# facebookresearch/hanabi_SAD

Hardware: AMD Instinct MI355X
Metric: hanabi_env_steps_per_sec (higher is better)
Workload: dtype u32

## Files before the change

hanabi_sad_amd/csrc/hsad_env.hip:

```cpp

#include <hip/hip_runtime.h>

#include <cstdarg>
#include <cstdlib>
#include <cstdio>
#include <cstring>
#include <new>
#include <string>
#include <vector>

#include "hsad.h"
#include "hsad_deal_fast.h"
#include "hsad_obs_row.h"
#include "hsad_planes.h"

namespace {

constexpr int kWave = 64;
constexpr int kMtN = 624;
constexpr int kMtM = 397;

struct EnvParams {
  static constexpr bool kScripted = false;
  int G, Gpad, P, H, A, F, F0, LAL, OB, OD, OL, OK, DECKW;
// ... 782 lines not shown
  return m;
}

template <int TH, class Ru>
__device__ __forceinline__ uint64_t legal_mask_of(int P, int H, int A, const uint32_t* s_st, int lane, int p, uint32_t pm,
                                                  const Ru& ru) {
  const uint32_t board = ST(PL_BOARD);
  const int cur = board_cur(board), info = board_info(board);
  uint64_t lm = 0;
  if (p == cur) {
    const uint32_t hw = ST(PLH(p));
    const int len = (hw >> 25) & 7;
    const uint64_t lenmask = (1ull << len) - 1ull;
    if (info < ru.MI) lm |= lenmask;
    lm |= lenmask << H;
    if (info > 0) {
      for (int o = 1; o < P; ++o) {
        int q = p + o;
        if (q >= P) q -= P;
        const uint32_t thw = ST(PLH(q));
        const int tl = (thw >> 25) & 7;
        uint32_t cm = 0, rm = 0;
#pragma unroll
        for (int i = 0; i < (TH ? TH : 5); ++i) {
          const int card = (thw >> (5 * i)) & 31;
          const int c = (card * 13) >> 6, r = card - 5 * c;
          if (i < tl) {
            cm |= 1u << perm_c(pm, c);
            rm |= 1u << r;
          }
        }
        lm |= (uint64_t)cm << (2 * H + (o - 1) * ru.C);
        lm |= (uint64_t)rm << (2 * H + (P - 1) * ru.C + (o - 1) * ru.R);
      }
    }
  }
  if (!lm) lm = 1ull << (A - 1);
  return lm;
}

template <int TP, int TH, bool V = false, bool FIXED = false>
__device__ __forceinline__ void build_rows(const EnvParams& ep, const uint32_t* s_st, int lane, int g, uint32_t* s_obs,
                                           uint32_t* s_legal, uint32_t* s_own, uint32_t greedy_rec, int p_begin,
                                           int p_step, uint32_t* s_lmask = nullptr) {
  const int P = TP ? TP : ep.P, H = TH ? TH : ep.H;
  const auto ru = RulesOf<V>::make(ep);
  const uint32_t CR = (uint32_t)ru.CR, RR = (uint32_t)ru.R;
  const uint32_t board = ST(PL_BOARD);
  const uint32_t misc = ST(PL_MISC);
  const int deck_size = (misc >> 8) & 63;
  const uint64_t disc = (uint64_t)ST(PL_DISC_LO) | ((uint64_t)ST(PL_DISC_HI) << 32);
  const uint32_t lastmv = ST(PL_LASTMV);
  const int info = board_info(board), life = board_life(board);
  const uint32_t F = (uint32_t)ep.F;

  for (int p = p_begin; p < P; p += p_step) {
    const uint32_t base = (uint32_t)(lane * P + p) * F;
    const uint32_t pm = ep.shuffle_color ? (ST(PLPERM(p)) & 0x7fffu) : kIdentityPerm;
    if constexpr (FIXED) {
      static_assert(TP > 0 && TH > 0 && !V, "fixed bit positions need a fixed game shape and the full rules");
      uint32_t hand[TP], kcp[TP], krp[TP], kh[TP];
#pragma unroll
      for (int o = 0; o < TP; ++o) {
        int q = p + o;
        if (q >= P) q -= P;
        hand[o] = ST(PLH(q));
        kcp[o] = ST(PLKCP(q));
        krp[o] = ST(PLKRP(q));
        kh[o] = ST(PLKH(q));
      }
      uint32_t row[ObsRowGeom<TP, TH>::NW];
      obs_row_assemble<TP, TH>(row, board, misc, disc, lastmv, greedy_rec, hand, kcp, krp, kh, p, pm, ep.sad != 0);
      obs_row_place<TP, TH>(row, base, ep.sad != 0, [s_obs](uint32_t w, uint32_t v) { atomicOr(&s_obs[w], v); });
    } else {
      uint32_t miss = 0;
#pragma unroll
      for (int o = 0; o < (TP ? TP : 5); ++o) {
        if (o >= P) break;
        int q = p + o;
        if (q >= P) q -= P;
        const uint32_t hw = ST(PLH(q));
        const int len = (hw >> 25) & 7;
        if (len < H) miss |= 1u << o;
        const uint32_t kcp = ST(PLKCP(q)), krp = ST(PLKRP(q)), kh = ST(PLKH(q));
#pragma unroll
        for (int i = 0; i < (TH ? TH : 5); ++i) {
          if (i < len) {
            if (o > 0) {
              const int card = (hw >> (5 * i)) & 31;
              const int c = (card * 13) >> 6, r = card - 5 * c;
              or_bit(s_obs, base + (uint32_t)((o * H + i) * ru.CR) + perm_c(pm, c) * RR + (uint32_t)r);
            }
            const uint32_t cp = (kcp >> (5 * i)) & 31u, rp = (krp >> (5 * i)) & 31u;
            const uint32_t h6 = (kh >> (6 * i)) & 63u;
            uint64_t m = 0;
#pragma unroll
            for (int c = 0; c < 5; ++c) m |= ((cp >> c) & 1u) ? ((uint64_t)rp << (perm_c(pm, c) * RR)) : 0ull;
            if (h6 & 7u) m |= 1ull << (CR + perm_c(pm, (int)(h6 & 7u) - 1));
            if (h6 >> 3) m |= 1ull << (CR + (uint32_t)ru.C + (h6 >> 3) - 1u);
            or_bits64(s_obs, base + (uint32_t)ep.OK + (uint32_t)((o * H + i) * ru.KS), m);
          }
        }
      }
      or_bits32(s_obs, base + (uint32_t)(P * H * ru.CR), miss);
      or_bits64(s_obs, base + (uint32_t)ep.OB, (1ull << deck_size) - 1ull);
      uint64_t bm = 0;
#pragma unroll
      for (int c = 0; c < 5; ++c) {
        const int f = board_fw(board, c);
        bm |= (f > 0) ? (1ull << (perm_c(pm, c) * RR + (uint32_t)f - 1u)) : 0ull;
      }
      bm |= (uint64_t)((1u << info) - 1u) << CR;
      bm |= (uint64_t)((1u << life) - 1u) << (CR + (uint32_t)ru.MI);
      or_bits64(s_obs, base + (uint32_t)(ep.OB + ep.DECKW), bm);
      uint64_t dm = 0;
#pragma unroll
      for (int c = 0; c < 5; ++c) {
        const uint32_t pc = perm_c(pm, c);
#pragma unroll
        for (int r = 0; r < 5; ++r) {
          const uint32_t n = cnt2(disc, c * 5 + r);
          const uint32_t roff = (r == 0) ? 0u : (1u + 2u * (uint32_t)r);
          dm |= (uint64_t)((1u << n) - 1u) << (pc * (uint32_t)ru.DW + roff);
        }
      }
      or_bits64(s_obs, base + (uint32_t)ep.OD, dm);
      or_bits64(s_obs, base + (uint32_t)ep.OL, encode_last_action(P, H, lastmv, p, pm, ru));
      if (ep.sad) or_bits64(s_obs, base + (uint32_t)ep.F0, encode_last_action(P, H, greedy_rec, p, pm, ru));
    }

    const uint64_t lm = legal_mask_of<TH>(P, H, ep.A, s_st, lane, p, pm, ru);
    or_bits64(s_legal, (uint32_t)(lane * P + p) * (uint32_t)ep.A, lm);
    ep.legal_bits[(size_t)g * P + p] = lm;
    if (ep.legal_out) ep.legal_out[(size_t)g * P + p] = lm;
    if (s_lmask) {
      s_lmask[(2 * p) * kWave + lane] = (uint32_t)lm;
      s_lmask[(2 * p + 1) * kWave + lane] = (uint32_t)(lm >> 32);
    }

    {
      const uint32_t hw = ST(PLH(p));
      const int len = (hw >> 25) & 7;
      uint32_t om = 0;
#pragma unroll
      for (int i = 0; i < (TH ? TH : 5); ++i) {
        const int card = (hw >> (5 * i)) & 31;
        const int c = (card * 13) >> 6, r = card - 5 * c;
        const int f = board_fw(board, c);
        if (i < len) om |= 1u << (3 * i + (r == f ? 0 : (r < f ? 1 : 2)));
      }
      or_bits32(s_own, (uint32_t)(lane * P + p) * (uint32_t)(3 * H), om);
      if (ep.own_bits) ep.own_bits[(size_t)g * P + p] = om;
    }
  }
}

__device__ __forceinline__ uint64_t public_counts(uint64_t disc, uint32_t board, uint64_t full) {
  uint64_t pc = full - disc;
#pragma unroll
  for (int c = 0; c < 5; ++c) {
    const int f = board_fw(board, c);
    for (int r = 0; r < f; ++r) pc -= (uint64_t)1 << (2 * (c * 5 + r));
  }
  return pc;
}

template <bool V>
__device__ void v0_fixup(const EnvParams& ep, const uint32_t* s_st, const uint32_t* s_obs, uint64_t active, int g0,
                         int lane_id) {
  const int P = ep.P, H = ep.H;
  const auto ru = RulesOf<V>::make(ep);
  const int per_row = P * H * ru.CR;
  while (active) {
    const int lg = __builtin_ctzll(active);
    active &= active - 1;
    const uint32_t board = s_st[PL_BOARD * kWave + lg];
    const uint64_t disc = (uint64_t)s_st[PL_DISC_LO * kWave + lg] | ((uint64_t)s_st[PL_DISC_HI * kWave + lg] << 32);
    const uint64_t pub = public_counts(disc, board, ru.full);
    for (int e = lane_id; e < P * per_row; e += kWave) {
      const int p = e / per_row;
      const int rem = e - p * per_row;
      const int slot = rem / ru.CR;
      const int j = rem - slot * ru.CR;
      const int o = slot / H, i = slot - o * H;
      int q = p + o;
      if (q >= P) q -= P;
      const uint32_t hw = s_st[PLH(q) * kWave + lg];
      if (i >= (int)((hw >> 25) & 7)) continue;
      const uint32_t bitpos = (uint32_t)(lg * P + p) * (uint32_t)ep.F + (uint32_t)ep.OK + (uint32_t)(slot * ru.KS + j);
      if (!get1(s_obs, bitpos)) continue;
      const uint32_t permw = ep.shuffle_color ? s_st[PLPERM(p) * kWave + lg] : kIdentityPermBoth;
      const uint32_t inv = permw >> 15;
      const uint32_t cp = (s_st[PLKCP(q) * kWave + lg] >> (5 * i)) & 31u;
      const uint32_t rp = (s_st[PLKRP(q) * kWave + lg] >> (5 * i)) & 31u;
      float total = 0.f;
      for (int c = 0; c < 5; ++c)
        if ((cp >> c) & 1u)
          for (int r = 0; r < 5; ++r)
            if ((rp >> r) & 1u) total += (float)cnt2(pub, c * 5 + r);
      const int pcol = j / ru.R, r = j - ru.R * pcol;
      const int real_c = (int)perm_c(inv, pcol);
      const float cnt = (float)cnt2(pub, real_c * 5 + r);
      const float v = (total > 0.f) ? cnt / total : 0.f;
      ep.priv_s[(size_t)(g0 + lg) * P * ep.F + (size_t)p * ep.F + ep.OK + slot * ru.KS + j] = v;
    }
  }
}

__device__ __forceinline__ void log_error(const EnvParams& ep, int g, int code) {
  if (atomicAdd(&ep.err[0], 1u) == 0u) {
    ep.err[1] = (uint32_t)g;
    ep.err[2] = (uint32_t)code;
  }
}

__device__ __forceinline__ int policy_pick(uint64_t seed, uint64_t game, uint64_t counter, int p, int stream,
                                           uint64_t mask) {
  const uint32_t h = policy_hash(seed, game, counter, (uint64_t)(p * 2 + stream));
  return df_select(mask, h % (uint32_t)__popcll(mask));
}
__device__ __forceinline__ uint64_t policy_key(uint64_t seed, uint64_t game, int p, int stream) {
  return mix64(seed ^ mix64(game * 0xD1342543DE82EF95ull + (uint64_t)(p * 2 + stream)));
}
__device__ __forceinline__ int policy_pick_keyed(uint64_t key, uint64_t counter, uint64_t mask, int nbits) {
  const uint32_t h = (uint32_t)(mix64(key + counter) >> 32);
  return df_select(mask, h % (uint32_t)__popcll(mask), nbits);
}

constexpr int kEnvThreads = 4 * kWave;

__device__ __forceinline__ void stream_rows(const EnvParams& ep, const uint32_t* s_obs, const uint32_t* s_legal, const uint32_t* s_own,
                                            int g0, int ng, int P, int H, int t, int n) {
  const size_t PF = (size_t)P * ep.F, PA = (size_t)P * ep.A, PO = (size_t)P * 3 * H;
  if (!ep.obs_f32) {
  } else if (ep.nt_stores) {
    stream_bits_f32_aligned<true>(s_obs, ep.priv_s + (size_t)g0 * PF, (uint32_t)(ng * PF), t, n);
  } else {
    stream_bits_f32_aligned<false>(s_obs, ep.priv_s + (size_t)g0 * PF, (uint32_t)(ng * PF), t, n);
  }
  stream_rows_packed(ep, s_obs, 0, ng * P, (size_t)g0 * P, t, n);
  stream_bits_f32_aligned<false>(s_legal, ep.legal + (size_t)g0 * PA, (uint32_t)(ng * PA), t, n);
  stream_bits_f32_aligned<false>(s_own, ep.own + (size_t)g0 * PO, (uint32_t)(ng * PO), t, n);
}

__device__ __forceinline__ unsigned stream_rows_delta(const EnvParams& ep, const uint32_t* s_obs, uint32_t* s_old, bool all,
                                                      const uint32_t* s_legal, const uint32_t* s_own, int g0, int ng, int P, int H,
                                                      int t, int n, bool count, int compact, unsigned& units) {
  const size_t PF = (size_t)P * ep.F, PA = (size_t)P * ep.A, PO = (size_t)P * 3 * H;
  unsigned stored = 0;
  bool by_lines = true;
  if (!ep.obs_f32) {
  } else if (compact && !all) {
    by_lines = false;
    float* out = ep.priv_s + (size_t)g0 * PF;
    if (compact == 2) {
      if (ep.nt_stores) {
        stored = stream_bits_f32_compact<true, 16>(s_obs, s_old, out, (uint32_t)(ng * PF), t, units);
      } else {
        stored = stream_bits_f32_compact<false, 16>(s_obs, s_old, out, (uint32_t)(ng * PF), t, units);
      }
    } else if (ep.nt_stores) {
      stored = stream_bits_f32_compact<true, 32>(s_obs, s_old, out, (uint32_t)(ng * PF), t, units);
    } else {
      stored = stream_bits_f32_compact<false, 32>(s_obs, s_old, out, (uint32_t)(ng * PF), t, units);
    }
  } else if (ep.nt_stores) {
    stored = stream_bits_f32_delta<true>(s_obs, s_old, all, ep.priv_s + (size_t)g0 * PF, (uint32_t)(ng * PF), t, n, count);
  } else {
    stored = stream_bits_f32_delta<false>(s_obs, s_old, all, ep.priv_s + (size_t)g0 * PF, (uint32_t)(ng * PF), t, n, count);
  }
  if (by_lines) units = stored;
  stream_rows_packed(ep, s_obs, 0, ng * P, (size_t)g0 * P, t, n);
  stream_bits_f32_aligned<false>(s_legal, ep.legal + (size_t)g0 * PA, (uint32_t)(ng * PA), t, n);
  stream_bits_f32_aligned<false>(s_own, ep.own + (size_t)g0 * PO, (uint32_t)(ng * PO), t, n);
  return stored;
}

__device__ __forceinline__ void clear_words(uint32_t* p, int nz, int t, int n) {
  uint4* z4 = reinterpret_cast<uint4*>(p);
  for (int k = t; k < (nz >> 2); k += n) z4[k] = make_uint4(0u, 0u, 0u, 0u);
  for (int k = (nz & ~3) + t; k < nz; k += n) p[k] = 0u;
}

__device__ __forceinline__ void clear_rows(const EnvParams& ep, uint32_t* s_obs, int t, int n) {
  const int nz = ep.obs_words + ep.legal_words + ep.own_words;
  uint4* z4 = reinterpret_cast<uint4*>(s_obs);
  for (int k = t; k < (nz >> 2); k += n) z4[k] = make_uint4(0u, 0u, 0u, 0u);
  for (int k = (nz & ~3) + t; k < nz; k += n) s_obs[k] = 0u;
}

struct LogicCarry {
  uint32_t* counter;
  const uint32_t* s_lmask;
  const uint64_t* pkey;
};
template <int TP, int TH>
constexpr bool kPolicyKeys = (TP == 2 && TH == 5);
template <int N>
__device__ __forceinline__ uint64_t carried_key(const uint64_t* k, int i) {
  uint64_t v = k[0];
#pragma unroll
  for (int j = 1; j < N; ++j) v = (i == j) ? k[j] : v;
  return v;
}
typedef __attribute__((address_space(3))) const uint32_t* LdsWordPtr;

// ... 425 lines not shown

  Rng rng;
  rng.mt = ep.mt + (size_t)g * kMtN;
  rng.draws = ST(PL_DRAWS);
  rng.la0 = ST(PL_LA0);
  rng.la1 = ST(PL_LA1);
  rng.la_n = (int)((ST(PL_MISC) >> 22) & 3u);
  rng.spos = (rng.draws + (uint32_t)rng.la_n) % (uint32_t)kMtN;
  rng.win = nullptr;
  rng.w_c = rng.w_n = 0;
  uint32_t greedy_rec = 0;
  float reward = 0.f;
  bool term = false;

  if (wave == 0) {
    env_logic<MODE, TP, TH, V>(ep, a_in, g_in, s_st, s_win, s_eps, lane, g, active, do_reset, rng, greedy_rec, reward, term, dbg_it);
    s_grec[lane] = greedy_rec;
  }
  __syncthreads();
  STAMP(2);

  Refill rf;
  refill_issue(rf, rng, active && wave == 0);
  if (active) build_rows<TP, TH, V>(ep, s_st, lane, g, s_obs, s_legal, s_own, s_grec[lane], wave, nwaves);
  STAMP(3);
  if (active && wave == 0) {
    refill_finish(rf, rng);
    ST(PL_DRAWS) = rng.draws;
    ST(PL_LA0) = rng.la0;
    ST(PL_LA1) = rng.la1;
    ST(PL_MISC) = (ST(PL_MISC) & ~(3u << 22)) | ((uint32_t)rng.la_n << 22);
    for (int pl = 0; pl < ep.npl; ++pl) ep.planes[(size_t)pl * ep.Gpad + g] = ST(pl);
  }
  __syncthreads();
  STAMP(4);

  const size_t PF = (size_t)P * ep.F, PA = (size_t)P * ep.A, PO = (size_t)P * 3 * H;
  if (MODE >= 1) {
    stream_rows(ep, s_obs, s_legal, s_own, g0, ng, P, H, tid, nthreads);
    if (valid && wave == 0) {
      for (int p = 0; p < P; ++p) ep.eps[(size_t)g * P + p] = __uint_as_float(ST(PLEPS(p)));
      ep.reward[g] = reward;
      ep.terminal[g] = term ? 1 : 0;
    }
    if (ep.kmode == 1) {
      __syncthreads();
      if (wave == 0) v0_fixup<V>(ep, s_st, s_obs, __ballot(valid), g0, lane);
    }
  } else {
    if (wave != 0) return;
    uint64_t todo = __ballot(active);
    const uint64_t todo_all = todo;
    while (todo) {
      const int lg = __builtin_ctzll(todo);
      todo &= todo - 1;
      if (ep.obs_f32) stream_bits_f32(s_obs, (uint32_t)(lg * PF), ep.priv_s + (size_t)(g0 + lg) * PF, (uint32_t)PF, lane);
      stream_rows_packed(ep, s_obs, lg * P, P, (size_t)(g0 + lg) * P, lane, kWave);
      stream_bits_f32(s_legal, (uint32_t)(lg * PA), ep.legal + (size_t)(g0 + lg) * PA, (uint32_t)PA, lane);
      stream_bits_f32(s_own, (uint32_t)(lg * PO), ep.own + (size_t)(g0 + lg) * PO, (uint32_t)PO, lane);
    }
    if (active)
      for (int p = 0; p < P; ++p) ep.eps[(size_t)g * P + p] = __uint_as_float(ST(PLEPS(p)));
    if (ep.kmode == 1) {
      __syncthreads();
      v0_fixup<V>(ep, s_st, s_obs, todo_all, g0, lane);
    }
  }
  STAMP(5);
}

template <int MODE, int TP, int TH, bool V = false>
__global__ __launch_bounds__(kEnvThreads) void env_kernel(EnvParams ep, const int64_t* __restrict__ a_in,
                                                          const int64_t* __restrict__ g_in) {
  env_body<MODE, TP, TH, V>(ep, a_in, g_in);
}

template <int TP, int TH, bool V = false>
__global__ __launch_bounds__(kEnvThreads) void env_step_scripted_kernel(ScriptedParams ep, const int64_t* __restrict__ a_in,
                                                                        const int64_t* __restrict__ g_in) {
  env_body<1, TP, TH, V>(ep, a_in, g_in);
}

__device__ __forceinline__ void rollout_stagger(const EnvParams& ep) {
  if (ep.stagger_ticks > 0) {
    unsigned k = blockIdx.x & 7u;
    if (ep.stagger_mode == 1) k = ((blockIdx.x >> 3) >> 5) & 3u;
    else if (ep.stagger_mode == 2) k = (blockIdx.x >> 3) & 3u;
    else if (ep.stagger_mode == 3) {
      unsigned hw;
      asm volatile("s_getreg_b32 %0, hwreg(HW_REG_HW_ID)" : "=s"(hw));
      k = (hw & 15u) >> 1;
    }
    const unsigned long long t_in = wall_clock64(), wait = (unsigned long long)k * (unsigned long long)ep.stagger_ticks;
    while (wall_clock64() - t_in < wait) __builtin_amdgcn_s_sleep(16);
  }
}

__device__ __forceinline__ unsigned pace_delay(const EnvParams& ep, unsigned long long s, int iter, unsigned t_own) {
  const long long num = (long long)iter * ep.pace_blocks - (long long)(s - ep.pace_base);
  const long long span = (long long)ep.n_iter * ep.pace_blocks;
  if (num < -span || num > span) return 0u;
  const int over_q8 = (int)((num * (long long)ep.pace_inv_q32) >> 24) - ep.pace_l0_q8;
  if (over_q8 <= 0) return 0u;
  t_own = min(t_own, 1u << 20);
  const unsigned long long d = ((unsigned long long)(unsigned)over_q8 * t_own) >> 8;
  return (unsigned)min(d, (unsigned long long)min(t_own >> 1, (unsigned)ep.pace_cap_ticks));
}

__device__ __forceinline__ unsigned long long pace_count(const EnvParams& ep) {
  int z = 0;
  unsigned long long one = 1ull;
  asm volatile("" : "+v"(z), "+v"(one));
  return __hip_atomic_fetch_add(ep.pace + z, one, __ATOMIC_RELAXED, __HIP_MEMORY_SCOPE_AGENT);
}

__device__ __forceinline__ void pace_sleep(unsigned ticks) {
  const unsigned long long t_in = wall_clock64();
  while (wall_clock64() - t_in < (unsigned long long)ticks) __builtin_amdgcn_s_sleep(16);
}

template <int TP, int TH, bool V = false>
__global__ __launch_bounds__(kEnvThreads) __attribute__((amdgpu_waves_per_eu(2, 2))) void env_rollout_kernel(EnvParams ep) {
  rollout_stagger(ep);
  unsigned long long pace_s = 0ull;
  unsigned pace_t0 = (unsigned)wall_clock64();
  const bool paced = ep.pace && ep.g_begin + (int)blockIdx.x * ep.gpw < ep.G;
#pragma clang loop unroll(disable)
  for (int iter = 0; iter < ep.n_iter; ++iter) {
    if (iter) __syncthreads();
    if (paced) {
      const unsigned now = (unsigned)wall_clock64(), t_own = now - pace_t0;
      pace_t0 = now;
      if (threadIdx.x == 0) {
        if (iter > 0) {
          const unsigned d = pace_delay(ep, pace_s, iter - 1, t_own);
          if (d) pace_sleep(d);
        }
        pace_s = pace_count(ep);
      }
    }
    int zero = 0;
    asm volatile("" : "+s"(zero));
    env_body<3, TP, TH, V>(ep, nullptr, nullptr, zero, iter);
  }
}

#ifdef HSAD_ENV_ROWBUILD_SCATTER
template <int TP, int TH>
constexpr bool kRowBuildFixed = false;
#else
template <int TP, int TH>
constexpr bool kRowBuildFixed = TP > 0 && TH > 0;
#endif

__device__ __forceinline__ unsigned wave_sum(unsigned v) {
  for (int o = kWave / 2; o > 0; o >>= 1) v += (unsigned)__shfl_xor((int)v, o, kWave);
  return v;
}

constexpr int kChainIn = 2, kChainOut = 4;
__device__ __forceinline__ uint4* chain_slice(const EnvParams& ep) {
  return reinterpret_cast<uint4*>(reinterpret_cast<uint32_t*>(ep.phase) + (size_t)blockIdx.x * ep.obs_words);
}

template <int TP, int TH>
__global__ __launch_bounds__(kEnvThreads) __attribute__((amdgpu_waves_per_eu(2, 2))) void env_rollout_pipe_kernel(EnvParams ep) {
  if constexpr (kRowBuildFixed<TP, TH>) asm volatile("" ::: "v175");
  rollout_stagger(ep);
  extern __shared__ __attribute__((aligned(16))) uint32_t smem[];
  uint32_t* s_st = smem;
  uint32_t* s_obs = s_st + ep.npl * kWave;
  uint32_t* s_legal = s_obs + ep.obs_words;
  uint32_t* s_own = s_legal + ep.legal_words;
  uint32_t* s_win = s_own + ep.own_words;
  uint32_t* s_grec = s_win + ep.win_words * kWave;
  float* s_eps = reinterpret_cast<float*>(s_grec + kWave);
  uint32_t* s_pace = s_grec + kWave + 128;
#define S_OBS1(z) (ep.delta ? s_pace + 4 + (z) : s_obs)

  const int tid = threadIdx.x;
  const int lane = tid & (kWave - 1);
  const int wave = tid >> 6;
  const int g0 = ep.g_begin + blockIdx.x * ep.gpw;
  const int ng = min(ep.gpw, ep.G - g0);
  if (ng <= 0) return;
  const int P = TP ? TP : ep.P, H = TH ? TH : ep.H;

  uint32_t act_counter = 0u;
  uint64_t pkey[kPolicyKeys<TP, TH> ? 2 * TP : 1] = {};
  if (wave == 0) {
    const int g = g0 + lane;
    if (lane < ng) {
      act_counter = ep.act_count[g];
      if constexpr (kPolicyKeys<TP, TH>) {
#pragma unroll
        for (int k = 0; k < 2 * TP; ++k) pkey[k] = policy_key(ep.policy_seed, (uint64_t)g, k >> 1, k & 1);
      }
      for (int p = 0; p < P; ++p) {
        const uint64_t lm = ep.legal_bits[(size_t)g * P + p];
        s_win[(2 * p) * kWave + lane] = (uint32_t)lm;
        s_win[(2 * p + 1) * kWave + lane] = (uint32_t)(lm >> 32);
      }
    }
    for (int pl0 = 0; pl0 < ep.npl; pl0 += 8) {
      uint32_t v[8];
#pragma unroll
      for (int j = 0; j < 8; ++j) v[j] = ep.planes[(size_t)min(pl0 + j, ep.npl - 1) * ep.Gpad + g];
#pragma unroll
      for (int j = 0; j < 8; ++j)
        if (pl0 + j < ep.npl) ST(pl0 + j) = v[j];
    }
  } else {
    clear_rows(ep, s_obs, lane, kWave);
    if (ep.delta & kChainIn) {
      const uint4* src = chain_slice(ep);
      uint4* dst = reinterpret_cast<uint4*>(S_OBS1(0));
      for (int k = lane; k < (ep.obs_words >> 2); k += kWave) dst[k] = src[k];
    }
    for (int k = lane; k < min(ep.n_eps, 128); k += kWave) s_eps[k] = ep.eps_list[k];
    if (lane == 0) s_pace[0] = 0u;
  }
  __syncthreads();

  unsigned pace_t0 = (unsigned)wall_clock64();
#pragma clang loop unroll(disable)
  for (int iter = 0; iter < ep.n_iter; ++iter) {
    int zero = 0;
    asm volatile("" : "+s"(zero));
    const int g = g0 + zero + lane;
    const bool valid = lane < ep.gpw && g < ep.G;
    const int dbg_it = iter;
    STAMP_START();
    unsigned long long pace_s = 0ull;
    if (ep.pace && tid == 0) pace_s = pace_count(ep);
    const unsigned pace_now = (unsigned)wall_clock64(), pace_t_own = pace_now - pace_t0;
    pace_t0 = pace_now;
    Rng rng = {};
    float reward = 0.f;
    bool term = false;
    if (wave == 0) {
      if (ep.dbg && ep.dbg_iters > 0) {
        asm volatile("s_waitcnt vmcnt(0)" ::: "memory");
        STAMP(1);
      }
      const uint32_t misc0 = ST(PL_MISC);
      const bool do_reset = valid && (!((misc0 >> 15) & 1u) || ((misc0 >> 14) & 1u));
      rng.mt = ep.mt + (size_t)g * kMtN;
      rng.draws = ST(PL_DRAWS);
      rng.la0 = ST(PL_LA0);
      rng.la1 = ST(PL_LA1);
      rng.la_n = (int)((misc0 >> 22) & 3u);
      rng.spos = (rng.draws + (uint32_t)rng.la_n) % (uint32_t)kMtN;
      uint32_t greedy_rec = 0;
      const LogicCarry carry = {&act_counter, s_win, pkey};
      env_logic<3, TP, TH, false, EnvParams, true>(ep, nullptr, nullptr, s_st, s_win, s_eps, lane, g, valid, do_reset, rng, greedy_rec, reward,
                                                   term, dbg_it, carry);
      s_grec[lane] = greedy_rec;
      STAMP(11);
    } else if (iter > 0) {
      if (ep.pace) {
        const unsigned d = (unsigned)__builtin_amdgcn_readfirstlane((int)s_pace[0]);
        if (d) pace_sleep(d);
      }
      uint32_t* s_obs1 = S_OBS1(zero);
      uint32_t* rows = (iter & 1) ? s_obs : s_obs1;
      uint32_t* prev = (iter & 1) ? s_obs1 : s_obs;
      const bool dbg_lines = ep.dbg && ep.dbg_iters > 0;
      int sl = lane;
      asm volatile("" : "+v"(sl));
      unsigned units = 0;
      const bool all = !ep.delta || (iter == 1 && !(ep.delta & kChainIn));
      unsigned stored = stream_rows_delta(ep, rows, prev, all, s_legal, s_own, g0, ng, P, H, sl, kWave, dbg_lines, ep.compact, units);
      clear_words(prev, ep.obs_words, sl, kWave);
      clear_words(s_legal, ep.legal_words + ep.own_words, sl, kWave);
      if (dbg_lines) {
        stored = wave_sum(stored);
        if (lane == 0) env_stamp(ep, dbg_it, 13, stored);
        unsigned long long* dbg_units = reinterpret_cast<unsigned long long*>(((uint64_t)ep.dbg_units_hi << 32) | ep.dbg_units_lo);
        if (dbg_units) {
          units = wave_sum(units);
          if (lane == 0)
            dbg_units[((size_t)(ep.g_begin / ep.gpw) + blockIdx.x) * ep.dbg_iters + (size_t)min(dbg_it, ep.dbg_iters - 1)] = units;
        }
      }
      STAMP_T(8, kWave);
    }
    __builtin_amdgcn_s_waitcnt(0xc07f);
    __syncthreads();
    STAMP(2);
    Refill rf;
    refill_issue(rf, rng, valid && wave == 0);
    if (valid)
      build_rows<TP, TH, false, kRowBuildFixed<TP, TH>>(ep, s_st, lane, g, (iter & 1) ? S_OBS1(zero) : s_obs, s_legal, s_own, s_grec[lane],
                                                        wave, 2, s_win);
    STAMP(3);
    if (valid && wave == 0) {
      refill_finish(rf, rng);
      ST(PL_DRAWS) = rng.draws;
      ST(PL_LA0) = rng.la0;
      ST(PL_LA1) = rng.la1;
      ST(PL_MISC) = (ST(PL_MISC) & ~(3u << 22)) | ((uint32_t)rng.la_n << 22);
      for (int p = 0; p < P; ++p) ep.eps[(size_t)g * P + p] = __uint_as_float(ST(PLEPS(p)));
      ep.reward[g] = reward;
      ep.terminal[g] = term ? 1 : 0;
      if (iter == ep.n_iter - 1) {
        for (int pl = 0; pl < ep.npl; ++pl) ep.planes[(size_t)pl * ep.Gpad + g] = ST(pl);
        ep.act_count[g] = act_counter;
      }
      if (ep.pace && lane == 0) {
        const unsigned d = iter > 0 ? pace_delay(ep, pace_s, iter, pace_t_own) : 0u;
        s_pace[0] = d;
        if (ep.dbg && ep.dbg_iters > 0) env_stamp(ep, dbg_it, 12, d);
      }
    }
    __syncthreads();
    STAMP(4);
  }
  const int dbg_it = ep.n_iter - 1;
  {
    uint32_t* s_obs1 = S_OBS1(0);
    const uint32_t* rows = (ep.n_iter & 1) ? s_obs : s_obs1;
    uint32_t* prev = (ep.n_iter & 1) ? s_obs1 : s_obs;
    const bool dbg_lines = ep.dbg && ep.dbg_iters > 0;
    unsigned units = 0;
    unsigned stored = stream_rows_delta(ep, rows, prev, !ep.delta || ep.n_iter == 1, s_legal, s_own, g0, ng, P, H, tid, ep.nthreads, dbg_lines,
                                        0, units);
    if (dbg_lines) {
      stored = wave_sum(stored);
      if (lane == 0) env_stamp(ep, dbg_it, 14 + wave, stored);
    }
    if (ep.delta & kChainOut) {
      const uint4* src = reinterpret_cast<const uint4*>(rows);
      uint4* dst = chain_slice(ep);
      for (int k = tid; k < (ep.obs_words >> 2); k += ep.nthreads) dst[k] = src[k];
    }
  }
  STAMP(5);
#undef S_OBS1
}

__device__ __forceinline__ void init_game(const EnvParams& ep, int g, int seed0, int period) {
  if (g >= ep.Gpad) return;
  for (int pl = 0; pl < ep.npl; ++pl) ep.planes[(size_t)pl * ep.Gpad + g] = 0u;
  if (g >= ep.G) return;
  ep.planes[(size_t)PL_MISC * ep.Gpad + g] = 0u;
  uint32_t* mt = ep.mt + (size_t)g * kMtN;
  uint32_t x = (uint32_t)(seed0 + (period > 0 ? g % period : g));
  mt[0] = x;
  for (int i = 1; i < kMtN; ++i) {
    x = 1812433253u * (x ^ (x >> 30)) + (uint32_t)i;
    mt[i] = x;
  }
  ep.act_count[g] = 0u;
}

__global__ void init_kernel(EnvParams ep) { init_game(ep, blockIdx.x * blockDim.x + threadIdx.x, ep.seed0, 0); }

__global__ void reseed_kernel(EnvParams ep, int seed0, int period) {
  init_game(ep, blockIdx.x * blockDim.x + threadIdx.x, seed0, period);
}

__global__ void policy_kernel(EnvParams ep, uint64_t seed, int64_t* __restrict__ a, int64_t* __restrict__ ga) {
  const int g = ep.g_begin + blockIdx.x * blockDim.x + threadIdx.x;
  if (g >= ep.g_begin + ep.g_count || g >= ep.G) return;
  const uint32_t counter = ep.act_count[g];
  ep.act_count[g] = counter + 1u;
  for (int p = 0; p < ep.P; ++p) {
    const uint64_t mask = ep.legal_bits[(size_t)g * ep.P + p];
    a[(size_t)g * ep.P + p] = policy_pick(seed, (uint64_t)g, (uint64_t)counter, p, 0, mask);
    if (ga) ga[(size_t)g * ep.P + p] = policy_pick(seed, (uint64_t)g, (uint64_t)counter, p, 1, mask);
  }
}

#define GP(pl) ep.planes[(size_t)(pl) * ep.Gpad + g]

__global__ void query_kernel(EnvParams ep, int32_t* __restrict__ out) {
  const int g = blockIdx.x * blockDim.x + threadIdx.x;
  if (g >= ep.G) return;
  const uint32_t board = GP(PL_BOARD), misc = GP(PL_MISC);
  int32_t* o = out + (size_t)g * HSAD_QUERY_WORDS;
  const bool started = misc_started(misc);
  o[HSAD_Q_TERMINATED] = misc_live(misc) ? 0 : 1;
  o[HSAD_Q_CUR_PLAYER] = board_cur(board);
  const int life = board_life(board);
  o[HSAD_Q_SCORE] = (life <= 0 && ep.bomb) ? 0 : board_fw_sum(board);
  o[HSAD_Q_LIFE] = life;
  o[HSAD_Q_INFO] = board_info(board);
  o[HSAD_Q_LAST_SCORE] = misc_last_score(misc);
  o[HSAD_Q_NUM_STEP] = misc_num_step(misc);
  o[HSAD_Q_DECK_SIZE] = misc_deck_size(misc);
  for (int c = 0; c < 5; ++c) o[HSAD_Q_FIREWORKS + c] = board_fw(board, c);
  o[HSAD_Q_RNG_DRAWS] = (int32_t)(GP(PL_DRAWS) & 0x7fffffffu);
  o[HSAD_Q_STARTED] = started ? 1 : 0;
  o[15] = 0;
}

__global__ void legal_query_kernel(EnvParams ep, const int32_t* __restrict__ uid, uint8_t* __restrict__ out) {
  const int g = blockIdx.x * blockDim.x + threadIdx.x;
  if (g >= ep.G) return;
  const uint32_t board = GP(PL_BOARD);
  const int cur = board_cur(board);
  const MoveDec m = decode_uid(uid[g], ep.P, ep.H, RulesOf<true>::make(ep));
  bool ok = false;
  if (m.type != 0 && cur >= 0) {
    if (m.type <= 2) {
      const int len = (GP(PLH(cur)) >> 25) & 7;
      ok = (m.idx < len) && !(m.type == 2 && board_info(board) >= ep.max_info);
    } else if (board_info(board) > 0 && m.off >= 1 && m.off < ep.P) {
      int q = cur + m.off;
      if (q >= ep.P) q -= ep.P;
      ok = hand_match_mask(GP(PLH(q)), m.type == 3, m.val) != 0;
    }
  }
  out[g] = ok ? 1 : 0;
}

__global__ void deck_history_kernel(EnvParams ep, uint8_t* __restrict__ out, int32_t* __restrict__ count) {
  const int g = blockIdx.x * blockDim.x + threadIdx.x;
  if (g >= ep.G) return;
  const uint32_t misc = GP(PL_MISC);
  const int n = misc_started(misc) ? ep.deck_max - misc_deck_size(misc) : 0;
  count[g] = ep.track_dh ? n : 0;
  for (int i = 0; i < 50; ++i) out[(size_t)g * 50 + i] = (ep.track_dh && i < n) ? ep.deck_hist[(size_t)g * 52 + i] : 0;
}

__global__ void export_state_kernel(EnvParams ep, int32_t* __restrict__ out, int words) {
  const int g = blockIdx.x * blockDim.x + threadIdx.x;
  const int P = ep.P;
  if (g >= ep.G) return;
  int32_t* o = out + (size_t)g * words;
  for (int i = 0; i < words; ++i) o[i] = 0;
  const uint64_t deck = (uint64_t)GP(PL_DECK_LO) | ((uint64_t)GP(PL_DECK_HI) << 32);
  const uint64_t disc = (uint64_t)GP(PL_DISC_LO) | ((uint64_t)GP(PL_DISC_HI) << 32);
  const uint32_t board = GP(PL_BOARD), misc = GP(PL_MISC), rec = GP(PL_LASTMV);
  for (int t = 0; t < 25; ++t) {
    o[t] = (int32_t)cnt2(deck, t);
    o[25 + t] = (int32_t)cnt2(disc, t);
  }
  for (int c = 0; c < 5; ++c) o[50 + c] = board_fw(board, c);
  o[55] = board_info(board);
  o[56] = board_life(board);
  o[57] = board_cur(board);
  o[58] = board_next(board);
  o[59] = board_turns(board);
  o[60] = misc_num_step(misc);
  o[61] = misc_deck_size(misc);
  const int type = rec & 7;
  o[62] = type;
  o[63] = -1;
  o[64] = o[65] = o[66] = o[67] = o[69] = o[70] = -1;
  if (type) {
    o[63] = (rec >> 3) & 7;
    if (type >= 3) {
      o[64] = (rec >> 6) & 7;
      if (type == 3) o[65] = (rec >> 9) & 7;
      if (type == 4) o[66] = (rec >> 12) & 7;
      o[68] = (rec >> 18) & 31;
    } else {
      o[67] = (rec >> 15) & 7;
      o[69] = (rec >> 23) & 7;
      o[70] = (rec >> 26) & 7;
      o[71] = (rec >> 29) & 1;
      o[72] = (rec >> 30) & 1;
    }
  }
  o[73] = (int32_t)(GP(PL_DRAWS) & 0x7fffffffu);
  o[74] = misc_last_score(misc);
  int base = 80;
  for (int p = 0; p < ep.P; ++p) {
    const uint32_t hw = GP(PLH(p)), kcp = GP(PLKCP(p)), krp = GP(PLKRP(p)), kh = GP(PLKH(p));
    const int len = (hw >> 25) & 7;
    for (int i = 0; i < ep.H; ++i) {
      int32_t* s = o + base + (p * ep.H + i) * 6;
      if (i < len) {
        s[0] = (hw >> (5 * i)) & 31;
        s[1] = (kcp >> (5 * i)) & 31;
        s[2] = (krp >> (5 * i)) & 31;
        s[3] = (int)((kh >> (6 * i)) & 7) - 1;
        s[4] = (int)((kh >> (6 * i + 3)) & 7) - 1;
      } else {
        s[0] = -1;
        s[3] = s[4] = -1;
      }
    }
  }
  base += ep.P * ep.H * 6;
  for (int p = 0; p < ep.P; ++p) {
    const uint32_t pw = misc_started(misc) ? GP(PLPERM(p)) : kIdentityPermBoth;
    for (int c = 0; c < 5; ++c) {
      o[base + p * 5 + c] = perm_c(pw & 0x7fffu, c);
      o[base + ep.P * 5 + p * 5 + c] = perm_c(pw >> 15, c);
// ... 792 lines not shown
```

hanabi_sad_amd/csrc/hsad_obs_row.h:

```cpp
#ifndef HSAD_OBS_ROW_H
#define HSAD_OBS_ROW_H

#include <stdint.h>

#if defined(__HIPCC__)
#define HSAD_OR_FN __host__ __device__ __forceinline__
#else
#define HSAD_OR_FN inline
#endif

template <int P, int H>
struct ObsRowGeom {
  static constexpr int C = 5, R = 5, CR = 25, KS = 35, DW = 10, MI = 8, ML = 3, DECK = 50;
  static constexpr int MISS = P * H * CR;
  static constexpr int OB = MISS + P;
  static constexpr int DECKW = DECK - P * H;
  static constexpr int OFW = OB + DECKW;
  static constexpr int OD = OFW + CR + MI + ML;
  static constexpr int LAL = P + 4 + P + C + R + H + H + CR + 2;
  static constexpr int OL = OD + DECK;
  static constexpr int OK = OL + LAL;
  static constexpr int F0 = OK + P * H * KS;
  static constexpr int FS = F0 + LAL;
  static constexpr int NW = (FS + 31) / 32;
// ... 25 lines not shown
    int tgt = rel + (int)((rec >> 6) & 7u);
    if (tgt >= P) tgt -= P;
    m |= 1ull << (P + 4 + tgt);
    m |= (uint64_t)((rec >> 18) & 31u) << (2 * P + 14);
  } else {
    m |= 1ull << (2 * P + 14 + H + ((rec >> 15) & 7u));
    m |= 1ull << (2 * P + 14 + 2 * H + ((pm >> (3u * ((rec >> 23) & 7u))) & 7u) * 5u + ((rec >> 26) & 7u));
  }
  if (type == 3) m |= 1ull << (2 * P + 4 + ((pm >> (3u * ((rec >> 9) & 7u))) & 7u));
  if (type == 4) m |= 1ull << (2 * P + 9 + ((rec >> 12) & 7u));
  if (type == 1) m |= (uint64_t)((rec >> 29) & 3u) << (2 * P + 39 + 2 * H);
  return m;
}

HSAD_OR_FN uint64_t obs_discards_identity(uint64_t disc) {
  const uint64_t r0 = 0x0000010040100401ull;
  const uint64_t k5 = 0x155ull * r0;
  const uint64_t r13 = 0x054ull * r0;
  const uint64_t r14 = 0x154ull * r0;
  const uint64_t lo = disc & k5, hi = (disc >> 1) & k5;
  const uint64_t ge1 = lo | hi, ge2 = hi, ge3 = lo & hi;
  return (ge1 & r0) | ((ge1 & r14) << 1) | ((ge2 & r0) << 1) | ((ge2 & r13) << 2) | ((ge3 & r0) << 2);
}

template <int P, int H>
HSAD_OR_FN void obs_row_assemble(ObsRow<P, H>& row, uint32_t board, uint32_t misc, uint64_t disc, uint32_t lastmv,
                                 uint32_t greedy, const uint32_t (&hand)[P], const uint32_t (&kcp)[P], const uint32_t (&krp)[P],
                                 const uint32_t (&kh)[P], int p, uint32_t pm, bool sad) {
  using Ge = ObsRowGeom<P, H>;
#if defined(__clang__)
#pragma unroll
#endif
  for (int k = 0; k < Ge::NW; ++k) row[k] = 0u;
  uint32_t pmc[5], sh5[5];
#if defined(__clang__)
#pragma unroll
#endif
  for (int c = 0; c < 5; ++c) {
    pmc[c] = (pm >> (3 * c)) & 7u;
    sh5[c] = 5u * pmc[c];
  }
  uint32_t len[P], kc[P];
#if defined(__clang__)
#pragma unroll
#endif
  for (int o = 0; o < P; ++o) {
    len[o] = (hand[o] >> 25) & 7u;
    kc[o] = kcp[o] & ((1u << (5u * len[o])) - 1u);
  }
  uint32_t hint_tab = (1u << 5) | (2u << 10) | (4u << 15) | (8u << 20) | (16u << 25);
  uint64_t dm = obs_discards_identity(disc);
  if (pm != kObsIdentityPerm) {
    const uint32_t each = 1u | (1u << 5) | (1u << 10) | (1u << 15) | (1u << 20);
#if defined(__clang__)
#pragma unroll
#endif
    for (int o = 0; o < P; ++o) {
      uint32_t t = 0;
#if defined(__clang__)
#pragma unroll
#endif
      for (int c = 0; c < 5; ++c) t |= ((kc[o] >> c) & each) << pmc[c];
      kc[o] = t;
    }
    hint_tab = 0;
    uint64_t t = 0;
#if defined(__clang__)
#pragma unroll
#endif
    for (int c = 0; c < 5; ++c) {
      hint_tab |= (1u << (5 * (c + 1))) << pmc[c];
      t |= ((dm >> (10 * c)) & 1023ull) << (2u * sh5[c]);
    }
    dm = t;
  }

  uint32_t miss = 0;
#if defined(__clang__)
#pragma unroll
#endif
  for (int o = 0; o < P; ++o) {
    const uint32_t hw = hand[o];
    miss |= (len[o] < (uint32_t)H ? 1u : 0u) << o;
    const uint32_t kr = krp[o], kk = kh[o] & ((1u << (6u * len[o])) - 1u);
#if defined(__clang__)
#pragma unroll
#endif
    for (int i = 0; i < H; ++i) {
      if (o > 0) {
        const uint32_t card = (hw >> (5 * i)) & 31u;
        const uint32_t c = (card * 13u) >> 6;
        const uint32_t pos = card + 5u * ((pm >> (3u * c)) & 7u) - 5u * c;
        obs_put(row, (o * H + i) * Ge::CR, Ge::CR, (uint32_t)i < len[o] ? 1u << pos : 0u);
      }
      const uint32_t cp = (kc[o] >> (5 * i)) & 31u, rp = (kr >> (5 * i)) & 31u, h6 = (kk >> (6 * i)) & 63u;
      const uint32_t spread = (((cp & 15u) * 0x1111u) & 0x8421u) | ((cp & 16u) << 16);
      const uint32_t hint = ((hint_tab >> (5u * (h6 & 7u))) & 31u) | (((1u << (h6 >> 3)) >> 1) << 5);
      obs_put(row, Ge::OK + (o * H + i) * Ge::KS, Ge::KS, (uint64_t)(rp * spread) | ((uint64_t)hint << Ge::CR));
    }
  }
  obs_put(row, Ge::MISS, P, miss);
  obs_put(row, Ge::OB, Ge::DECKW, (1ull << ((misc >> 8) & 63u)) - 1ull);
  uint32_t fw = 0;
#if defined(__clang__)
#pragma unroll
#endif
  for (int c = 0; c < 5; ++c) fw |= ((1u << ((board >> (3 * c)) & 7u)) >> 1) << sh5[c];
  obs_put(row, Ge::OFW, Ge::CR, fw);
  const uint32_t info = (board >> 15) & 15u, life = (board >> 19) & 3u;
  obs_put(row, Ge::OFW + Ge::CR, Ge::MI + Ge::ML, ((1u << info) - 1u) | (((1u << life) - 1u) << Ge::MI));
  obs_put(row, Ge::OD, Ge::DECK, dm);
  obs_put(row, Ge::OL, Ge::LAL, obs_last_action<P, H>(lastmv, p, pm));
  if (sad) obs_put(row, Ge::F0, Ge::LAL, obs_last_action<P, H>(greedy, p, pm));
}

HSAD_OR_FN uint32_t obs_funnel(uint32_t hi, uint32_t lo, uint32_t sh) {
#if defined(__HIP_DEVICE_COMPILE__)
  return __builtin_amdgcn_alignbit(hi, lo, sh);
#endif
  return (uint32_t)((((uint64_t)hi << 32) | (uint64_t)lo) >> (sh & 31u));
}

template <int NW>
HSAD_OR_FN uint32_t obs_at(const uint32_t (&row)[NW], const int k) {
  return k < NW ? row[k < NW ? k : 0] : 0u;
}

template <int P, int H, class OrFn>
HSAD_OR_FN void obs_row_place(const ObsRow<P, H>& row, uint32_t base, bool sad, OrFn or_word) {
  using Ge = ObsRowGeom<P, H>;
  constexpr int K0 = Ge::F0 >> 5, K1 = Ge::FS >> 5;
  const uint32_t s = base & 31u, sh = (32u - s) & 31u;
  const uint32_t wb = (base >> 5) - (s == 0u ? 1u : 0u);
  const uint32_t last = (base + (uint32_t)(sad ? Ge::FS : Ge::F0) - 1u) >> 5;
  constexpr int Z = (H * Ge::CR) >> 5;
  static_assert(Z >= 1 && Z < K0, "the first image word written is an interior one");
#if defined(__clang__)
#pragma unroll
#endif
  for (int k = Z; k <= K0; ++k) or_word(wb + k, obs_funnel(obs_at(row, k), k > Z ? obs_at(row, k - 1) : 0u, sh));
  if (sad) {
#if defined(__clang__)
#pragma unroll
#endif
    for (int k = K0 + 1; k <= K1; ++k) or_word(wb + k, obs_funnel(obs_at(row, k), obs_at(row, k - 1), sh));
    const uint32_t x = wb + K1 + 1;
    or_word(x < last ? x : last, obs_funnel(obs_at(row, K1 + 1), obs_at(row, K1), sh));
  } else {
    const uint32_t x = wb + K0 + 1;
    or_word(x < last ? x : last, obs_funnel(obs_at(row, K0 + 1), obs_at(row, K0), sh));
  }
}

#endif
```

Baseline: 2.322 billion.

## Prebuild observation rows in wave 0 before barrier, place after sync

For the TP=2, TH=5 fixed configuration, wave 0 now assembles the shifted observation row images, legal masks and own-card bits in registers right after env_logic, before the block barrier. It also finishes the RNG refill and the global output stores before that barrier, so after the sync it only ORs the prepared images into shared memory. This takes row assembly out of the post-barrier critical section, which the streaming waves otherwise wait on. The cost is higher register pressure from holding the row images across the barrier, and the v175 register reservation is dropped for this path.

New measurement: 2.304 billion. About the same (-0.8%).

```diff
diff --git a/hanabi_sad_amd/csrc/hsad_env.hip b/hanabi_sad_amd/csrc/hsad_env.hip
--- a/hanabi_sad_amd/csrc/hsad_env.hip
+++ b/hanabi_sad_amd/csrc/hsad_env.hip
@@ -958,6 +958,74 @@
       or_bits32(s_own, (uint32_t)(lane * P + p) * (uint32_t)(3 * H), om);
       if (ep.own_bits) ep.own_bits[(size_t)g * P + p] = om;
     }
+  }
+}
+
+template <int TP, int TH>
+struct PreRows {
+  uint32_t img[TP][ObsRowShifted<TP, TH>::NS];
+  uint64_t lm[TP];
+  uint32_t om[TP];
+};
+
+template <int TP, int TH>
+__device__ __forceinline__ void rows_prebuild(const EnvParams& ep, const uint32_t* s_st, int lane, int g, uint32_t greedy_rec,
+                                              uint32_t* s_lmask, bool store_legal_bits, PreRows<TP, TH>& pr) {
+  constexpr int P = TP;
+  const auto ru = RulesOf<false>::make(ep);
+  const uint32_t board = ST(PL_BOARD);
+  const uint32_t misc = ST(PL_MISC);
+  const uint64_t disc = (uint64_t)ST(PL_DISC_LO) | ((uint64_t)ST(PL_DISC_HI) << 32);
+  const uint32_t lastmv = ST(PL_LASTMV);
+  const uint32_t F = (uint32_t)ep.F;
+#pragma unroll
+  for (int p = 0; p < TP; ++p) {
+    const uint32_t base = (uint32_t)(lane * TP + p) * F;
+    const uint32_t pm = ep.shuffle_color ? (ST(PLPERM(p)) & 0x7fffu) : kIdentityPerm;
+    uint32_t hand[TP], kcp[TP], krp[TP], kh[TP];
+#pragma unroll
+    for (int o = 0; o < TP; ++o) {
+      const int q = p + o < TP ? p + o : p + o - TP;
+      hand[o] = ST(PLH(q));
+      kcp[o] = ST(PLKCP(q));
+      krp[o] = ST(PLKRP(q));
+      kh[o] = ST(PLKH(q));
+    }
+    uint32_t row[ObsRowGeom<TP, TH>::NW];
+    obs_row_assemble<TP, TH>(row, board, misc, disc, lastmv, greedy_rec, hand, kcp, krp, kh, p, pm, ep.sad != 0);
+    obs_row_shift<TP, TH>(pr.img[p], row, base & 31u);
+
+    const uint64_t lm = legal_mask_of<TH>(TP, TH, ep.A, s_st, lane, p, pm, ru);
+    pr.lm[p] = lm;
+    if (store_legal_bits) ep.legal_bits[(size_t)g * TP + p] = lm;
+    if (ep.legal_out) ep.legal_out[(size_t)g * TP + p] = lm;
+    s_lmask[(2 * p) * kWave + lane] = (uint32_t)lm;
+    s_lmask[(2 * p + 1) * kWave + lane] = (uint32_t)(lm >> 32);
+
+    const uint32_t hw = hand[0];
+    const int len = (hw >> 25) & 7;
+    uint32_t om = 0;
+#pragma unroll
+    for (int i = 0; i < TH; ++i) {
+      const int card = (hw >> (5 * i)) & 31;
+      const int c = (card * 13) >> 6, r = card - 5 * c;
+      const int f = board_fw(board, c);
+      if (i < len) om |= 1u << (3 * i + (r == f ? 0 : (r < f ? 1 : 2)));
+    }
+    pr.om[p] = om;
+    if (ep.own_bits) ep.own_bits[(size_t)g * TP + p] = om;
+  }
+}
+
+template <int TP, int TH>
+__device__ __forceinline__ void rows_place(const EnvParams& ep, int lane, const PreRows<TP, TH>& pr, uint32_t* s_obs, uint32_t* s_legal,
+                                           uint32_t* s_own) {
+#pragma unroll
+  for (int p = 0; p < TP; ++p) {
+    const uint32_t r = (uint32_t)(lane * TP + p);
+    obs_row_or<TP, TH>(pr.img[p], r * (uint32_t)ep.F, ep.sad != 0, [s_obs](uint32_t w, uint32_t v) { atomicOr(&s_obs[w], v); });
+    or_bits64(s_legal, r * (uint32_t)ep.A, pr.lm[p]);
+    or_bits32(s_own, r * (uint32_t)(3 * TH), pr.om[p]);
   }
 }
 
@@ -1689,6 +1757,21 @@
 template <int TP, int TH>
 constexpr bool kRowBuildFixed = TP > 0 && TH > 0;
 #endif
+#ifdef HSAD_ENV_ROWBUILD_PHASE_B
+template <int TP, int TH>
+constexpr bool kRowPrebuild = false;
+#else
+template <int TP, int TH>
+constexpr bool kRowPrebuild = kRowBuildFixed<TP, TH> && TP == 2 && TH == 5;
+#endif
+template <int TP, int TH, bool ON>
+struct PreRowsOf {
+  using type = PreRows<TP, TH>;
+};
+template <int TP, int TH>
+struct PreRowsOf<TP, TH, false> {
+  struct type {};
+};
 
 __device__ __forceinline__ unsigned wave_sum(unsigned v) {
   for (int o = kWave / 2; o > 0; o >>= 1) v += (unsigned)__shfl_xor((int)v, o, kWave);
@@ -1700,9 +1783,25 @@
   return reinterpret_cast<uint4*>(reinterpret_cast<uint32_t*>(ep.phase) + (size_t)blockIdx.x * ep.obs_words);
 }
 
+#define PIPE_FINISH_ITERATION(rf)                                                                             \
+  do {                                                                                                        \
+    refill_finish(rf, rng);                                                                                   \
+    ST(PL_DRAWS) = rng.draws;                                                                                 \
+    ST(PL_LA0) = rng.la0;                                                                                     \
+    ST(PL_LA1) = rng.la1;                                                                                     \
+    ST(PL_MISC) = (ST(PL_MISC) & ~(3u << 22)) | ((uint32_t)rng.la_n << 22);                                   \
+    for (int p = 0; p < P; ++p) ep.eps[(size_t)g * P + p] = __uint_as_float(ST(PLEPS(p)));                    \
+    ep.reward[g] = reward;                                                                                    \
+    ep.terminal[g] = term ? 1 : 0;                                                                            \
+    if (iter == ep.n_iter - 1) {                                                                              \
+      for (int pl = 0; pl < ep.npl; ++pl) ep.planes[(size_t)pl * ep.Gpad + g] = ST(pl);                       \
+      ep.act_count[g] = act_counter;                                                                          \
+    }                                                                                                         \
+  } while (0)
+
 template <int TP, int TH>
 __global__ __launch_bounds__(kEnvThreads) __attribute__((amdgpu_waves_per_eu(2, 2))) void env_rollout_pipe_kernel(EnvParams ep) {
-  if constexpr (kRowBuildFixed<TP, TH>) asm volatile("" ::: "v175");
+  if constexpr (kRowBuildFixed<TP, TH> && !kRowPrebuild<TP, TH>) asm volatile("" ::: "v175");
   rollout_stagger(ep);
   extern __shared__ __attribute__((aligned(16))) uint32_t smem[];
   uint32_t* s_st = smem;
@@ -1775,6 +1874,8 @@
     Rng rng = {};
     float reward = 0.f;
     bool term = false;
+    typename PreRowsOf<TP, TH, kRowPrebuild<TP, TH>>::type pre;
+    unsigned pre_delay = 0u;
     if (wave == 0) {
       if (ep.dbg && ep.dbg_iters > 0) {
         asm volatile("s_waitcnt vmcnt(0)" ::: "memory");
@@ -1792,8 +1893,18 @@
       const LogicCarry carry = {&act_counter, s_win, pkey};
       env_logic<3, TP, TH, false, EnvParams, true>(ep, nullptr, nullptr, s_st, s_win, s_eps, lane, g, valid, do_reset, rng, greedy_rec, reward,
                                                    term, dbg_it, carry);
-      s_grec[lane] = greedy_rec;
+      if constexpr (!kRowPrebuild<TP, TH>) s_grec[lane] = greedy_rec;
       STAMP(11);
+      if constexpr (kRowPrebuild<TP, TH>) {
+        Refill rf;
+        refill_issue(rf, rng, valid);
+        if (valid) {
+          rows_prebuild<TP, TH>(ep, s_st, lane, g, greedy_rec, s_win, iter == ep.n_iter - 1, pre);
+          PIPE_FINISH_ITERATION(rf);
+          if (ep.pace && lane == 0 && iter > 0) pre_delay = pace_delay(ep, pace_s, iter, pace_t_own);
+        }
+        STAMP(5);
+      }
     } else if (iter > 0) {
       if (ep.pace) {
         const unsigned d = (unsigned)__builtin_amdgcn_readfirstlane((int)s_pace[0]);
@@ -1825,29 +1936,27 @@
     __builtin_amdgcn_s_waitcnt(0xc07f);
     __syncthreads();
     STAMP(2);
-    Refill rf;
-    refill_issue(rf, rng, valid && wave == 0);
-    if (valid)
-      build_rows<TP, TH, false, kRowBuildFixed<TP, TH>>(ep, s_st, lane, g, (iter & 1) ? S_OBS1(zero) : s_obs, s_legal, s_own, s_grec[lane],
-                                                        wave, 2, s_win);
-    STAMP(3);
-    if (valid && wave == 0) {
-      refill_finish(rf, rng);
-      ST(PL_DRAWS) = rng.draws;
-      ST(PL_LA0) = rng.la0;
-      ST(PL_LA1) = rng.la1;
-      ST(PL_MISC) = (ST(PL_MISC) & ~(3u << 22)) | ((uint32_t)rng.la_n << 22);
-      for (int p = 0; p < P; ++p) ep.eps[(size_t)g * P + p] = __uint_as_float(ST(PLEPS(p)));
-      ep.reward[g] = reward;
-      ep.terminal[g] = term ? 1 : 0;
-      if (iter == ep.n_iter - 1) {
-        for (int pl = 0; pl < ep.npl; ++pl) ep.planes[(size_t)pl * ep.Gpad + g] = ST(pl);
-        ep.act_count[g] = act_counter;
+    if constexpr (kRowPrebuild<TP, TH>) {
+      if (valid && wave == 0) rows_place<TP, TH>(ep, lane, pre, (iter & 1) ? S_OBS1(zero) : s_obs, s_legal, s_own);
+      STAMP(3);
+      if (ep.pace && tid == 0) {
+        s_pace[0] = pre_delay;
+        if (ep.dbg && ep.dbg_iters > 0) env_stamp(ep, dbg_it, 12, pre_delay);
       }
-      if (ep.pace && lane == 0) {
-        const unsigned d = iter > 0 ? pace_delay(ep, pace_s, iter, pace_t_own) : 0u;
-        s_pace[0] = d;
-        if (ep.dbg && ep.dbg_iters > 0) env_stamp(ep, dbg_it, 12, d);
+    } else {
+      Refill rf;
+      refill_issue(rf, rng, valid && wave == 0);
+      if (valid)
+        build_rows<TP, TH, false, kRowBuildFixed<TP, TH>>(ep, s_st, lane, g, (iter & 1) ? S_OBS1(zero) : s_obs, s_legal, s_own, s_grec[lane],
+                                                          wave, 2, s_win);
+      STAMP(3);
+      if (valid && wave == 0) {
+        PIPE_FINISH_ITERATION(rf);
+        if (ep.pace && lane == 0) {
+          const unsigned d = iter > 0 ? pace_delay(ep, pace_s, iter, pace_t_own) : 0u;
+          s_pace[0] = d;
+          if (ep.dbg && ep.dbg_iters > 0) env_stamp(ep, dbg_it, 12, d);
+        }
       }
     }
     __syncthreads();
@@ -1874,6 +1983,7 @@
   }
   STAMP(5);
 #undef S_OBS1
+#undef PIPE_FINISH_ITERATION
 }
 
 __device__ __forceinline__ void init_game(const EnvParams& ep, int g, int seed0, int period) {
diff --git a/hanabi_sad_amd/csrc/hsad_obs_row.h b/hanabi_sad_amd/csrc/hsad_obs_row.h
--- a/hanabi_sad_amd/csrc/hsad_obs_row.h
+++ b/hanabi_sad_amd/csrc/hsad_obs_row.h
@@ -201,4 +201,48 @@
   }
 }
 
-#endif
+template <int P, int H>
+struct ObsRowShifted {
+  using Ge = ObsRowGeom<P, H>;
+  static constexpr int Z = (H * Ge::CR) >> 5, K0 = Ge::F0 >> 5, K1 = Ge::FS >> 5;
+  static constexpr int NS = K1 + 2 - Z;
+  static_assert(Z >= 1 && Z < K0, "the first image word written is an interior one");
+};
+
+template <int P, int H>
+using ObsRowImage = uint32_t[ObsRowShifted<P, H>::NS];
+
+template <int P, int H>
+HSAD_OR_FN void obs_row_shift(ObsRowImage<P, H>& img, const ObsRow<P, H>& row, uint32_t s) {
+  using Sh = ObsRowShifted<P, H>;
+  const uint32_t sh = (32u - (s & 31u)) & 31u;
+#if defined(__clang__)
+#pragma unroll
+#endif
+  for (int k = Sh::Z; k <= Sh::K1 + 1; ++k) img[k - Sh::Z] = obs_funnel(obs_at(row, k), k > Sh::Z ? obs_at(row, k - 1) : 0u, sh);
+}
+
+template <int P, int H, class OrFn>
+HSAD_OR_FN void obs_row_or(const ObsRowImage<P, H>& img, uint32_t base, bool sad, OrFn or_word) {
+  using Ge = ObsRowGeom<P, H>;
+  using Sh = ObsRowShifted<P, H>;
+  const uint32_t wb = (base >> 5) - ((base & 31u) == 0u ? 1u : 0u);
+  const uint32_t last = (base + (uint32_t)(sad ? Ge::FS : Ge::F0) - 1u) >> 5;
+#if defined(__clang__)
+#pragma unroll
+#endif
+  for (int k = Sh::Z; k <= Sh::K0; ++k) or_word(wb + k, img[k - Sh::Z]);
+  if (sad) {
+#if defined(__clang__)
+#pragma unroll
+#endif
+    for (int k = Sh::K0 + 1; k <= Sh::K1; ++k) or_word(wb + k, img[k - Sh::Z]);
+    const uint32_t x = wb + Sh::K1 + 1;
+    or_word(x < last ? x : last, img[Sh::K1 + 1 - Sh::Z]);
+  } else {
+    const uint32_t x = wb + Sh::K0 + 1;
+    or_word(x < last ? x : last, img[Sh::K0 + 1 - Sh::Z]);
+  }
+}
+
+#endif
```
